# jtdaugherty/flux

Measured on AMD Instinct MI355X. Metric: Msamples/sec on demo2.yml (fixed spp), higher is better.
Workload: dtype f64

## Files before the change

flux_amd/csrc/flux_plan.h:

```cpp
#pragma once
#include <stddef.h>
#include <stdint.h>

#include "flux_device.h"

#ifndef FLUX_BLOCK_THREADS
#define FLUX_BLOCK_THREADS 64
#endif
#ifndef FLUX_WPE_SPLIT
#define FLUX_WPE_SPLIT 5
#endif
#ifndef FLUX_HITQ_MIN_TAKE
#define FLUX_HITQ_MIN_TAKE 32
#endif

namespace flux {

constexpr int kGlossExpSlots = 4;

constexpr int kQueueDoubles = 9;
constexpr int kQueueBytesPerWave = (kQueueDoubles * 64) * 8 + 2 * 64 * 4;
constexpr int kHitQDoubles = 7;
constexpr int kHitQInts = 3;
constexpr int kHitQBytesPerSlot = kHitQDoubles * 8 + kHitQInts * 4;
enum HitQField : uint32_t {
    kHitQOx = 0, kHitQOy = 2, kHitQOz = 4, kHitQDx = 6, kHitQDy = 8, kHitQDz = 10, kHitQT = 12,
    kHitQHitDepth = 14,
    kHitQSample = 15,
    kHitQList = 16,
};
constexpr uint32_t kHitQDwordsPerSlot = kHitQBytesPerSlot / 4;
constexpr uint32_t hitq_entry_dword(uint32_t C, uint32_t k) { return (C - 1u - k) * kHitQDwordsPerSlot; }
constexpr bool hitq_admits_phase_a(uint32_t C, uint32_t nhit) { return nhit + 64u <= C; }

constexpr size_t kTputEntryBytes = 24;
constexpr size_t kTputTableMaxBytes = (size_t)4 << 20;
constexpr uint32_t tput_index(uint32_t list_bits, uint32_t ml) { return (1u << list_bits) | ml; }
size_t tput_table_bytes(const RenderParams &p, int *bits = nullptr);

enum KernelCopy { kCopyStrict = 0, kCopyFast = 1, kCopyFastDiel = 2 };
KernelCopy kernel_copy(const RenderParams &p, int math);

struct LaunchPlan {
    int kernel = -1;
    unsigned block = 64;
    uint64_t blocks = 0;
    size_t lds = 0;
    unsigned waves_per_pixel = 1;
    int lds_scene = 0;
    int hq_cap = 0, hq_th = 0, hq_bits = 0;
    int copy = kCopyFast;
    int tris = 0;
    int typ = 0;
    int max32 = 0;
};
LaunchPlan plan_render(const RenderParams &p, int variant, int math);

size_t lane_stacks_lds(int math, size_t depth, bool tris, size_t bvh_stack, size_t lanes);
size_t shade_rays_lds(const RenderParams &p, int math);

}
```

flux_amd/csrc/launch_plan.cpp:

```cpp
#include <algorithm>
#include <cstdlib>

#include "flux_plan.h"
#include "../../include/flux_abi.h"

namespace flux {

KernelCopy kernel_copy(const RenderParams &p, int math) {
    if (math == FLUX_MATH_STRICT) return kCopyStrict;
    return p.has_diel ? kCopyFastDiel : kCopyFast;
}

size_t lane_stacks_lds(int math, size_t depth, bool tris, size_t bvh_stack, size_t lanes) {
    return (math == FLUX_MATH_STRICT ? depth * 4 * lanes * sizeof(double) : 0) + (tris ? bvh_stack * lanes * sizeof(int) : 0);
}

size_t shade_rays_lds(const RenderParams &p, int math) {
    return lane_stacks_lds(math, (size_t)p.max_depth, p.n_tris > 0, (size_t)p.bvh_stack, 64);
}

static bool split_typ(const RenderParams &p) {
    return p.n_sph <= 32 && p.glossy_long == 0 && p.unit_dirs == 1 && p.self_skip == 1 && p.env_short == 1 && p.n_uni == 1 &&
           p.fsph32 != nullptr && p.n_dsk == 0 && p.n_box == 0 && p.has_diel == 0 && (p.n_gloss_exp == 0 || p.gx_stride != 0);
}
// ... 7 lines not shown
    while (K * 2u <= (unsigned)FLUX_MAX_WAVES_PER_PIXEL && (uint64_t)K * 2u * FLUX_MIN_SAMPLES_PER_WAVE <= N) K *= 2u;
    return K;
}

static size_t split_scene_lds(const RenderParams &p) {
    return (size_t)hit_records(p) * sizeof(DevHitRec) + (size_t)p.n_sph * sizeof(DevScanSphere);
}
static bool split_serves(const RenderParams &p) { return p.n_tris == 0 && p.n_sph <= 64 && split_scene_lds(p) <= 16384; }

static bool plan_hitq(const RenderParams &p, unsigned K, size_t scene_lds, uint32_t &cap, uint32_t &th, int &bits) {
    if (p.glossy_long != 0 || p.has_diel != 0) return false;
    const size_t granules = (size_t)128 * K / (4 * FLUX_WPE_SPLIT);
    const size_t per_wave = granules * 1280 > scene_lds + 96 ? (granules * 1280 - scene_lds - 96) / K : 0;
    cap = (uint32_t)(per_wave / kHitQBytesPerSlot) & ~1u;
    if (const char *e = std::getenv("FLUX_SPLIT_HITQ_CAP")) cap = std::min(cap, (uint32_t)std::max(0, std::atoi(e)) & ~1u);
    th = cap > 64u + FLUX_HITQ_MIN_TAKE ? std::min(64u, cap - 64u) : FLUX_HITQ_MIN_TAKE;
    if (const char *e = std::getenv("FLUX_SPLIT_HITQ_TAKE_AT")) th = (uint32_t)std::max(1, std::min(64, std::atoi(e)));
    bits = 1;
    while ((1 << bits) < hit_records(p)) ++bits;
    return cap >= 64u + th && bits * p.max_depth <= 32;
}

size_t tput_table_bytes(const RenderParams &p, int *bits_out) {
    uint32_t cap, th;
    int bits;
    if (p.nsamp < 64u || p.max_depth < 2 || !split_serves(p) || !plan_hitq(p, waves_per_pixel(p.nsamp), split_scene_lds(p), cap, th, bits))
        return 0;
    const int list_bits = bits * (p.max_depth - 1);
    if (list_bits + 1 > 24) return 0;
    const size_t bytes = ((size_t)2 << list_bits) * kTputEntryBytes;
    if (bytes > kTputTableMaxBytes) return 0;
    if (bits_out) *bits_out = bits;
    return bytes;
}

LaunchPlan plan_render(const RenderParams &p, int variant, int math) {
    LaunchPlan L;
    L.copy = kernel_copy(p, math);
    const bool fast = L.copy != kCopyStrict;
    const uint32_t N = p.nsamp;
    const uint64_t npix = (uint64_t)p.num_rows * (uint64_t)p.img_w;
    if (npix == 0 || p.set_count <= 0) return L;
    if (variant == FLUX_KERNEL_DEFAULT) variant = N >= 256u ? FLUX_KERNEL_SPLIT : FLUX_KERNEL_REFILL;
    if (N < 64u) variant = FLUX_KERNEL_STATIC;
    const uint32_t lpp = N >= 64u ? 64u : N;
    const uint32_t ppw = 64u / lpp;
    uint64_t waves = (npix + ppw - 1) / ppw;
    if (variant != FLUX_KERNEL_STATIC && p.num_sets == (uint32_t)p.img_w)
        waves = 8ull * ((uint64_t)(p.set_count / 8) * (uint64_t)p.num_rows +
                        ((uint64_t)(p.set_count % 8) * (uint64_t)p.num_rows + 7u) / 8u);
    unsigned K = variant != FLUX_KERNEL_STATIC ? waves_per_pixel(N) : 1u;
    const bool tris = p.n_tris > 0;
    if (!fast && variant != FLUX_KERNEL_STATIC)
        while (K > 1u && lane_stacks_lds(math, (size_t)p.max_depth, tris, (size_t)p.bvh_stack, 64 * K) > 60 * 1024) K /= 2u;
    const unsigned block = (variant == FLUX_KERNEL_STATIC) ? FLUX_BLOCK_THREADS : 64u * K;
    const unsigned wpb = (variant == FLUX_KERNEL_STATIC) ? block / 64 : 1u;
    L.blocks = (waves + wpb - 1) / wpb;
    if (fast && variant != FLUX_KERNEL_STATIC && tris && p.bvh_stack > 0) {
        L.block = 64;
        size_t lds4 = (size_t)(p.bvh4_stack > 0 ? p.bvh4_stack : 1) * 64 * sizeof(int);
        const size_t scene4 = (size_t)hit_records(p) * sizeof(DevHitRec) + (size_t)p.n_mats * sizeof(DevMaterial) +
                              (size_t)p.n_sph * sizeof(DevScanSphere);
        const bool lds_scene4 = lds4 + scene4 <= 7680;
        if (lds_scene4) lds4 += scene4;
        if (p.nodes4 != nullptr && p.bvh4_stack <= FLUX_BVH_WIDE_MAX_STACK) {
            L.kernel = 4;
            L.lds = lds4;
            L.lds_scene = lds_scene4 ? 1 : 0;
            L.typ = bvh4_typ(p, lds_scene4) ? 1 : 0;
        } else {
            L.kernel = 3;
            L.lds = (size_t)p.bvh_stack * 64 * sizeof(int);
        }
        return L;
    }
    const size_t scene_lds = split_scene_lds(p);
    if (fast && variant == FLUX_KERNEL_SPLIT && split_serves(p)) {
        L.kernel = 2;
        L.block = block;
        L.waves_per_pixel = K;
        L.lds = (size_t)kQueueBytesPerWave * K + scene_lds;
        L.typ = split_typ(p) ? 1 : 0;
        L.max32 = p.n_sph <= 32 ? 1 : 0;
        uint32_t cap, th;
        int bits;
        if (plan_hitq(p, K, scene_lds, cap, th, bits)) {
            L.hq_cap = (int)cap;
            L.hq_th = (int)th;
            L.hq_bits = bits;
            L.lds = (size_t)cap * kHitQBytesPerSlot * K + scene_lds;
        }
        return L;
    }
    L.kernel = variant == FLUX_KERNEL_STATIC ? 0 : 1;
    L.block = block;
    L.waves_per_pixel = variant == FLUX_KERNEL_STATIC ? 1 : K;
    L.lds = lane_stacks_lds(math, (size_t)p.max_depth, tris, (size_t)p.bvh_stack, block);
    L.tris = tris ? 1 : 0;
    return L;
}

}
```

flux_amd/csrc/render_body.inc:

```

#undef FLUX_STAGE
#if FLUX_FAST
#define FLUX_STAGE() __builtin_amdgcn_sched_barrier(0)
#else
#define FLUX_STAGE() ((void)0)
#endif

struct Ray {
    double ox, oy, oz, dx, dy, dz;
};

typedef const __attribute__((address_space(4))) RenderParams *ParamsInKernarg;
static_assert(sizeof(DevMaterial) % 16 == 0, "the bounce-weight records behind the materials are read as double2");
__device__ __forceinline__ const RenderParams &relaunder_params(uint32_t tick) {
    ParamsInKernarg p = (ParamsInKernarg)__builtin_amdgcn_kernarg_segment_ptr();
    asm("" : "+s"(p) : "s"(tick));
    return *(const RenderParams *)p;
}

__device__ __forceinline__ unsigned long long ballot64(bool b) { return __builtin_amdgcn_ballot_w64(b); }
__device__ __forceinline__ bool any64(bool b) { return __builtin_amdgcn_ballot_w64(b) != 0ull; }
__device__ __forceinline__ bool all64(bool b) { return __builtin_amdgcn_ballot_w64(!b) == 0ull; }

typedef double flux_d2 __attribute__((ext_vector_type(2)));
// ... 765 lines not shown
#else
    return best;
#endif
}

__device__ __forceinline__ V3 to_unit_hemi(double2 p, double inv_e1) {
#if FLUX_FAST
    double sin_phi, cos_phi;
    fastmath::fsincos2pi(p.x, sin_phi, cos_phi);
    FLUX_STAGE();
    const double cos_theta = fastmath::fpow_pos(1.0 - p.y, inv_e1);
    FLUX_STAGE();
    const double sin_theta = fastmath::fsqrt(1.0 - cos_theta * cos_theta);
    return mk(sin_theta * cos_phi, sin_theta * sin_phi, cos_theta);
#else
    double phi = 2.0 * kPi * p.x;
    double sin_phi, cos_phi;
    sincos(phi, &sin_phi, &cos_phi);
    double cos_theta = pow(1.0 - p.y, inv_e1);
    double sin_theta = sqrt(1.0 - cos_theta * cos_theta);
    return normalize(mk(sin_theta * cos_phi, sin_theta * sin_phi, cos_theta));
#endif
}

__device__ __forceinline__ bool dielectric_dir(V3 n, V3 d, double ri, double u, V3 &wi) {
    const double ln = sqrt(n.x * n.x + n.y * n.y + n.z * n.z), ld = sqrt(d.x * d.x + d.y * d.y + d.z * d.z);
    const V3 nh = mk(n.x / ln, n.y / ln, n.z / ln), dh = mk(d.x / ld, d.y / ld, d.z / ld);
    double c = -(dh.x * nh.x + dh.y * nh.y + dh.z * nh.z);
    double eta = ri;
    V3 m = nh;
    if (!(c > 0.0)) {
        eta = 1.0 / ri;
        m = mk(-nh.x, -nh.y, -nh.z);
        c = -c;
    }
    const double k = 1.0 - (1.0 - c * c) / (eta * eta);
    double F = 1.0, ct = 0.0;
    if (!(k < 0.0)) {
        ct = sqrt(k);
        const double rs = (c - eta * ct) / (c + eta * ct);
        const double rp = (eta * c - ct) / (eta * c + ct);
        F = (rs * rs + rp * rp) / 2.0;
    }
    if (u <= F) {
        const double c2 = 2.0 * c;
        wi = mk(dh.x + c2 * m.x, dh.y + c2 * m.y, dh.z + c2 * m.z);
        return true;
    }
    const double a = c / eta - ct;
    wi = mk(dh.x / eta + a * m.x, dh.y / eta + a * m.y, dh.z / eta + a * m.z);
    return false;
}

struct Path {
    Ray r;
    int depth;
    int nb;
    double2 sq;
#if FLUX_FAST
    double tr, tg, tb;
    int self;
    int mat;
#endif
};
__device__ __forceinline__ int path_self(const Path &p) {
#if FLUX_FAST
    return p.self;
#else
    return -1;
#endif
}

__device__ __forceinline__ void path_begin(Path &p) {
    p.depth = 1;
    p.nb = 0;
#if FLUX_FAST
    p.tr = p.tg = p.tb = 1.0;
    p.self = -1;
    p.mat = 0;
#endif
}

#if FLUX_FAST
template <bool STATS, bool TRIS, bool TYP = false, bool FIRST = false>
__device__ __forceinline__ void fast_bounce(const RenderParams &P, Path &p, uint32_t set, uint32_t i, int hit, int slot, double t, V3 n,
                                            V3 d, V3 pt, int kind, double fr, double fg, double fb, double m_inv_e1, double ax, double az,
                                            bool unit_n, bool convex, bool is_tri, Stats &st, int cz) {
    (void)cz;
    const bool p_glossy_long = TYP ? false : P.glossy_long != 0;
    const bool p_unit_dirs = TYP ? true : P.unit_dirs != 0;
    const bool p_self_skip = TYP ? true : P.self_skip != 0;
    V3 wi;
    double scale = 1.0;
    const bool matte = kind == kMatMatte;
    FLUX_CENSUS(P, 6 + cz);
#if FLUX_DIEL
    if (!TYP && kind == kMatDielectric) {
        const char *hbase = !TRIS ? reinterpret_cast<const char *>(set_rows_of(P, set).hemi)
                                  : reinterpret_cast<const char *>(P.hemi + (size_t)set * P.max_depth * P.nsamp * 4);
        const double u = gather_global<double>(hbase, ((uint32_t)(p.depth - 1) * P.nsamp + i) * 32u + 16u);
        if (dielectric_dir(n, d, m_inv_e1, u, wi)) {
            if (STATS) st.c[10]++;
            fr = fg = fb = 1.0;
        } else {
            if (STATS) st.c[11]++;
        }
    } else
#endif
    {
        V3 w = n;
        if (!matte) {
            const double ndotwo = -dot(n, d);
            w = mk(d.x + n.x * ndotwo * 2.0, d.y + n.y * ndotwo * 2.0, d.z + n.z * ndotwo * 2.0);
        }
        if (kind == kMatReflective) {
            if (STATS) st.c[4]++;
            wi = w;
        } else {
            double hx, hy, hz;
            if (matte) {
                FLUX_CENSUS(P, 7 + cz);
                if (STATS) st.c[2]++;
                const size_t N = P.nsamp;
                const char *hbase = !TRIS ? reinterpret_cast<const char *>(set_rows_of(P, set).hemi)
                                                             : reinterpret_cast<const char *>(P.hemi + (size_t)set * P.max_depth * N * 4);
                const uint32_t hoff = ((uint32_t)(p.depth - 1) * (uint32_t)N + i) * 32u;
                const double2 hxy = gather_global_d2(hbase, hoff);
                hx = hxy.x;
                hy = hxy.y;
                hz = gather_global<double>(hbase, hoff + 16u);
                if (TRIS && is_tri) scale = 1.0 / kInvPi;
            } else {
                FLUX_CENSUS(P, 8 + cz);
                if (STATS) st.c[3]++;
                const char *gbase = !TRIS ? reinterpret_cast<const char *>(set_rows_of(P, set).gloss)
                                                             : reinterpret_cast<const char *>(P.gloss + (size_t)set * P.nsamp * 4);
                const double2 cs = gather_global_d2(gbase, i * 32u);
                double cos_theta, sin_theta;
                if (!TRIS && (TYP || P.gx_stride != 0)) {
                    const uint32_t xoff = __umul24(i, (uint32_t)P.gx_stride) + (uint32_t)gather_global<int32_t>(P.gx_off, (uint32_t)hit << 2);
                    const double2 csx = gather_global_d2(set_rows_of(P, set).glossx, xoff);
                    cos_theta = csx.x;
                    sin_theta = csx.y;
                } else {
                    cos_theta = fastmath::fexp2_tab(m_inv_e1 * gather_global<double>(gbase, i * 32u + 16u), P.exp2c);
                    sin_theta = fastmath::fsqrt(1.0 - cos_theta * cos_theta);
                }
                hx = sin_theta * cs.x;
                hy = sin_theta * cs.y;
                hz = cos_theta;
            }
            const V3 b1 = normalize(cross(mk(ax, 1.0, az), w));
            const V3 b2 = cross(b1, w);
            const double c1 = matte ? hy : hx, c2 = matte ? hx : hy;
            const V3 q = mk(c1 * b1.x + c2 * b2.x, c1 * b1.y + c2 * b2.y, c1 * b1.z + c2 * b2.z);
            const V3 hw = mk(hz * w.x, hz * w.y, hz * w.z);
            const V3 wi0 = mk(q.x + hw.x, q.y + hw.y, q.z + hw.z);
            if (matte) {
                wi = wi0;
                if (p_glossy_long) {
                    const V3 wn = normalize(wi0);
                    wi = unit_n ? wi0 : wn;
                }
            } else {
                const bool below = dot(n, wi0) < 0.0;
                wi = wi0;
                if (ballot64(below) != 0ull)
                    wi = mk(below ? hw.x - q.x : wi0.x, below ? hw.y - q.y : wi0.y, below ? hw.z - q.z : wi0.z);
                if (p_glossy_long) {
                    const double rdotwi = dot(w, wi), ndotwi = dot(n, wi);
                    const DevMaterial &Ml = P.mats[is_tri ? P.tris[slot].mat : P.frec[hit].orig_id];
                    const double e = Ml.exponent;
                    const int parity = Ml.exp_parity;
                    double lobe = fastmath::fpow_pos(fabs(rdotwi), e);
                    if (e == 0.0) lobe = 1.0;
                    if (rdotwi < 0.0) lobe = parity == 1 ? lobe : (parity == 2 ? -lobe : __builtin_nan(""));
                    if (rdotwi != rdotwi) lobe = rdotwi;
                    const double pdf = lobe * ndotwi;
                    fr *= lobe;
                    fg *= lobe;
                    fb *= lobe;
                    scale = ndotwi / pdf;
                }
            }
        }
    }
    if (p_unit_dirs) {
        const double ss = matte ? 1.0 : __builtin_fma(-0.5, dot(wi, wi), 1.5);
        wi = mk(wi.x * ss, wi.y * ss, wi.z * ss);
    }
    p.self = (p_self_skip && convex && __double2hiint(t) < 0x408f4000 && dot(n, wi) >= 0.0) ? hit : -1;
    if (FIRST) {
        p.tr = fr * scale;
        p.tg = fg * scale;
        p.tb = fb * scale;
    } else {
        p.tr *= fr * scale;
        p.tg *= fg * scale;
        p.tb *= fb * scale;
    }
    p.nb++;
    p.depth++;
    p.r.ox = pt.x;
    p.r.oy = pt.y;
    p.r.oz = pt.z;
    p.r.dx = wi.x;
    p.r.dy = wi.y;
    p.r.dz = wi.z;
}

template <bool LDS_SCENE>
__device__ __forceinline__ int analytic_hit_fields(const RenderParams &P, const Ray &r, int hit, double t, const char *frec_lds, V3 &n,
                                                   int &kind, bool &unit_n, bool &convex, double &fr, double &fg, double &fb,
                                                   double &m_inv_e1, double &ax, double &az) {
    (void)frec_lds;
    const DevHitRec R = *reinterpret_cast<const DevHitRec *>((LDS_SCENE ? frec_lds : reinterpret_cast<const char *>(P.frec)) +
                                                              (uint32_t)hit * (uint32_t)sizeof(DevHitRec));
    kind = R.mat_kind;
    unit_n = R.unit_normal != 0;
    fr = R.fr; fg = R.fg; fb = R.fb; m_inv_e1 = R.inv_e1;
    ax = R.ax; az = R.az;
    const V3 ns = mk(((r.ox - R.cx) + t * r.dx) * R.inv_rad, ((r.oy - R.cy) + t * r.dy) * R.inv_rad,
                     ((r.oz - R.cz) + t * r.dz) * R.inv_rad);
    const bool sph = R.shape_kind == kShapeSphere;
    n = mk(sph ? ns.x : R.cx, sph ? ns.y : R.cy, sph ? ns.z : R.cz);
    convex = sph && R.inv_rad > 0.0;
    return R.orig_id;
}

template <bool STATS, bool TRIS, bool LDS_SCENE = false, bool TYP = false, bool FIRST = false, bool BOUNCE = true, bool FACING = false>
__device__ __forceinline__ bool shade_hit_fast(const RenderParams &P, Path &p, uint32_t set, uint32_t i, int hit, int slot, double t,
                                               double &Lr, double &Lg, double &Lb, Stats &st, int cz, const char *frec_lds = nullptr,
                                               int facing = 0) {
    (void)frec_lds;
    (void)facing;
    (void)cz;
    int bounce = 0;
    const bool is_tri = TRIS && slot >= 0;
    const V3 d = mk(p.r.dx, p.r.dy, p.r.dz);
    const V3 pt = mk(p.r.ox + t * d.x, p.r.oy + t * d.y, p.r.oz + t * d.z);
    V3 n = mk(0.0, 0.0, 1.0);
    int kind = kMatEmissive;
    bool unit_n = true;
    bool convex = false;
    double fr = 0.0, fg = 0.0, fb = 0.0, m_inv_e1 = 0.0, ax = 0.0, az = 0.0;
    if (hit < 0) {
        Lr = P.bgr;
        Lg = P.bgg;
        Lb = P.bgb;
        if (STATS) st.c[6]++;
    } else {
        if (is_tri) {
            const DevTri &T = P.tris[slot];
            const DevMaterial &Mt = P.mats[T.mat];
            p.mat = T.mat;
            n = mk(T.nx, T.ny, T.nz);
            kind = Mt.kind;
            fr = Mt.fr; fg = Mt.fg; fb = Mt.fb; m_inv_e1 = Mt.inv_e1;
            ax = kind == kMatMatte ? 0.0034 : 0.00424;
            az = kind == kMatMatte ? 0.0071 : 0.00764;
        } else {
            p.mat = analytic_hit_fields<LDS_SCENE>(P, p.r, hit, t, frec_lds, n, kind, unit_n, convex, fr, fg, fb, m_inv_e1, ax, az);
        }
        if (kind == kMatEmissive) {
            if (STATS) st.c[5]++;
            bool front;
            if (FACING && ballot64(!facing_known(facing)) == 0ull) {
                const DevHitRec &R = *reinterpret_cast<const DevHitRec *>(frec_lds + (uint32_t)hit * (uint32_t)sizeof(DevHitRec));
                front = facing_front(facing, reinterpret_cast<const int *>(&R.inv_rad)[1]);
            } else {
                front = ((n.x * -1.0) * d.x + (n.y * -1.0) * d.y + (n.z * -1.0) * d.z) > 0.0;
            }
            Lr = fr;
            Lg = fg;
            Lb = fb;
            if (ballot64(!front) != 0ull) {
                Lr = front ? fr : 0.0;
                Lg = front ? fg : 0.0;
                Lb = front ? fb : 0.0;
            }
        } else {
            bounce = 1;
        }
    }
    asm("" : "+v"(bounce));
    if (BOUNCE && bounce) {
        fast_bounce<STATS, TRIS, TYP, FIRST>(P, p, set, i, hit, slot, t, n, d, pt, kind, fr, fg, fb, m_inv_e1, ax, az, unit_n, convex, is_tri, st,
                                            cz);
    }
    return bounce != 0;
}

template <bool STATS, bool TYP>
__device__ __forceinline__ void bounce_parked_hit(const RenderParams &P, Path &p, uint32_t set, uint32_t i, int hit, double t, Stats &st,
                                                  int cz, const char *frec_lds) {
    const V3 d = mk(p.r.dx, p.r.dy, p.r.dz);
    const V3 pt = mk(p.r.ox + t * d.x, p.r.oy + t * d.y, p.r.oz + t * d.z);
    V3 n;
    int kind;
    bool unit_n, convex;
    double fr, fg, fb, m_inv_e1, ax, az;
    p.mat = analytic_hit_fields<true>(P, p.r, hit, t, frec_lds, n, kind, unit_n, convex, fr, fg, fb, m_inv_e1, ax, az);
    fast_bounce<STATS, false, TYP, false>(P, p, set, i, hit, -1, t, n, d, pt, kind, fr, fg, fb, m_inv_e1, ax, az, unit_n, convex, false, st, cz);
}
#endif

template <bool STATS, bool TRIS, bool TWO_PHASE = false, bool LDS_SCENE = false, bool TYP = false>
__device__ __forceinline__ bool shade_hit(const RenderParams &P, Path &p, uint32_t set, uint32_t i, int hit,
                                          int slot, double t, double *stk, int stk_stride, double &Lr,
                                          double &Lg, double &Lb, Stats &st, int cz = 0, const char *frec_lds = nullptr,
                                          const char *mats_lds = nullptr) {
    (void)cz;
    (void)frec_lds;
    (void)mats_lds;
#if FLUX_FAST
    if (TWO_PHASE) return shade_hit_fast<STATS, TRIS>(P, p, set, i, hit, slot, t, Lr, Lg, Lb, st, cz);
#endif
    if (hit < 0) {
        Lr = P.bgr;
        Lg = P.bgg;
        Lb = P.bgb;
        if (STATS) st.c[6]++;
        return false;
    }
    const bool is_tri = TRIS && slot >= 0;
    const V3 d = mk(p.r.dx, p.r.dy, p.r.dz);
    const V3 pt = mk(p.r.ox + t * d.x, p.r.oy + t * d.y, p.r.oz + t * d.z);
    V3 n;
#if FLUX_FAST
    int kind;
    bool unit_n = true;
    bool convex = false;
    double fr, fg, fb, m_inv_e1, ax, az;
    if (is_tri) {
        const DevTri &T = P.tris[slot];
        const DevMaterial &Mt = LDS_SCENE ? *reinterpret_cast<const DevMaterial *>(mats_lds + (uint32_t)T.mat * (uint32_t)sizeof(DevMaterial))
                                          : P.mats[T.mat];
        p.mat = T.mat;
        n = mk(T.nx, T.ny, T.nz);
        kind = Mt.kind;
        fr = Mt.fr; fg = Mt.fg; fb = Mt.fb; m_inv_e1 = Mt.inv_e1;
        ax = kind == kMatMatte ? 0.0034 : 0.00424;
        az = kind == kMatMatte ? 0.0071 : 0.00764;
    } else {
        const DevHitRec R = *reinterpret_cast<const DevHitRec *>((LDS_SCENE ? frec_lds : reinterpret_cast<const char *>(P.frec)) +
                                                                  (uint32_t)hit * (uint32_t)sizeof(DevHitRec));
        kind = R.mat_kind;
        p.mat = R.orig_id;
        unit_n = R.unit_normal != 0;
        fr = R.fr; fg = R.fg; fb = R.fb; m_inv_e1 = R.inv_e1;
        ax = R.ax; az = R.az;
        const V3 ns = mk(((p.r.ox - R.cx) + t * d.x) * R.inv_rad, ((p.r.oy - R.cy) + t * d.y) * R.inv_rad,
                         ((p.r.oz - R.cz) + t * d.z) * R.inv_rad);
        const bool sph = R.shape_kind == kShapeSphere;
        n = mk(sph ? ns.x : R.cx, sph ? ns.y : R.cy, sph ? ns.z : R.cz);
        convex = sph && R.inv_rad > 0.0;
    }
    if (kind == kMatEmissive) {
        if (STATS) st.c[5]++;
        const bool front = ((n.x * -1.0) * d.x + (n.y * -1.0) * d.y + (n.z * -1.0) * d.z) > 0.0;
        Lr = front ? fr : 0.0;
        Lg = front ? fg : 0.0;
        Lb = front ? fb : 0.0;
        return false;
    }
#else
    const DevShape *S = P.shapes + (is_tri ? 0 : hit);
// ... 462 lines not shown
template <bool TYP>
__device__ __forceinline__ void scan_shapes_primary(const RenderParams &P, const Ray &r, unsigned long long cand_mask,
                                                    unsigned long long in_mask, double in_t0, bool valid, unsigned long long valid_m,
                                                    int &best, double &tb) {
    (void)valid;
    (void)valid_m;
    int best_id = -1;
    const double tmin = P.t_min;
    int j0 = 0;
    if (P.n_pln > 0) {
        const DevScanPlane &S = P.fpln[0];
        const double num = (S.px - r.ox) * S.nx + (S.py - r.oy) * S.ny + (S.pz - r.oz) * S.nz;
        const double den = r.dx * S.nx + r.dy * S.ny + r.dz * S.nz;
        const double t = num / den;
        best = t > tmin ? P.n_sph : -1;
        best_id = S.id;
        tb = t;
        j0 = 1;
    }
    for (int j = j0; j < P.n_pln; ++j) {
        const DevScanPlane &S = P.fpln[j];
        const double num = (S.px - r.ox) * S.nx + (S.py - r.oy) * S.ny + (S.pz - r.oz) * S.nz;
        const double den = r.dx * S.nx + r.dy * S.ny + r.dz * S.nz;
        const double t = num / den;
        if (t > tmin && (best < 0 || t < tb)) {
            best = P.n_sph + j;
            best_id = S.id;
            tb = t;
        }
    }
    if (!TYP) {
        scan_disks(P, r, tmin, best, best_id, tb);
        scan_boxes(P, r, tmin, best, best_id, tb);
    }
    const double rs = 1.0, ux = r.dx, uy = r.dy, uz = r.dz, len = 1.0;
    const bool zflat = r.dz == 0.0, any_zflat = any64(zflat);
    for (int pass = 0; pass < 2; ++pass) {
        unsigned long long todo = pass == 0 ? (cand_mask & ~in_mask) : in_mask;
        if (pass == 1 && todo && (valid_m & ~(ballot64(best >= 0) & ballot64(tb <= in_t0))) == 0ull) todo &= todo - 1;
        while (todo) {
            const int k = __builtin_ctzll(todo);
            todo &= todo - 1;
            const DevScanSphere S = P.fsph[k];
            FLUX_TRIP(P, 13);
            FLUX_CENSUS(P, 1);
            const double tx = r.ox - S.px, ty = r.oy - S.py, tz = r.oz - S.pz;
            const double hb = sphere_hb(tx, ty, tz, ux, uy, uz);
            const double c = __builtin_fma(tx, tx, __builtin_fma(ty, ty, __builtin_fma(tz, tz, -S.rr)));
            if (pass == 1) {
                const double tu = tb * len;
                const double g = __builtin_fma(tu, __builtin_fma(2.0, hb, tu), c);
                if ((valid_m & ~(ballot64(best >= 0) & ballot64(g < -1e-7 * S.rr))) == 0ull) continue;
            }
            const double dq = __builtin_fma(hb, hb, -c);
            const double e = fastmath::fsqrt_nonneg(__builtin_fmax(dq, 0.0));
            double t = (-hb - e) * rs;
            if (!(t > tmin)) t = (-hb + e) * rs;
            bool ok = dq >= 0.0 && t > tmin;
            if (any_zflat) {
                if (zflat && box_z_nan_miss(P, r, k)) ok = false;
            }
            if (ok) {
                bool take = best < 0 || t < tb;
                if (!take && t == tb) take = best >= P.n_sph ? P.frec[k].orig_id < best_id : k < best;
                if (take) {
                    best = k;
                    tb = t;
                }
            }
        }
    }
}

__device__ __forceinline__ double lds_dword_pair(const uint32_t *p) { return __hiloint2double((int)p[1], (int)p[0]); }
__device__ __forceinline__ void lds_dword_pair_store(uint32_t *p, double v) {
    p[0] = (uint32_t)__double2loint(v);
    p[1] = (uint32_t)__double2hiint(v);
}

__device__ __forceinline__ uint32_t *hitq_entry(uint32_t *pool, uint32_t C, uint32_t k) {
    return reinterpret_cast<uint32_t *>(reinterpret_cast<char *>(pool) + __umul24(C - 1u - k, (uint32_t)kHitQBytesPerSlot));
}

template <bool STATS, bool MAX32, bool TYP, bool HQ = false>
__global__ __launch_bounds__(64 * FLUX_MAX_WAVES_PER_PIXEL, FLUX_WPE_SPLIT) void render_split_kernel(const RenderParams P0, int hq_cap, int hq_th,
                                                                                                  int hq_bits) {
    (void)hq_cap;
    (void)hq_th;
    (void)hq_bits;
    const RenderParams &P = P0;
    extern __shared__ double lds_stack[];
    __shared__ double part[FLUX_MAX_WAVES_PER_PIXEL][3];
    const int tid = threadIdx.x;
    const uint32_t lane = tid & 63;
    const uint32_t N = P.nsamp;
    const uint32_t K = blockDim.x >> 6, sub = (uint32_t)__builtin_amdgcn_readfirstlane(tid >> 6);
    const uint32_t s_lo = (uint32_t)((uint64_t)N * sub / K), s_hi = (uint32_t)((uint64_t)N * (sub + 1) / K);
    const int n_rec = TYP ? P.n_sph + P.n_pln + P.n_dsk : hit_records(P);
    const size_t scene_lds_bytes = (size_t)n_rec * sizeof(DevHitRec) + (size_t)P.n_sph * sizeof(DevScanSphere);
    double *q = lds_stack + scene_lds_bytes / 8 + (size_t)sub * (HQ ? (size_t)hq_cap * kHitQBytesPerSlot / 8 : kQueueBytesPerWave / 8);
    int *qi = reinterpret_cast<int *>(q + (size_t)kQueueDoubles * 64);
    const char *const frec_lds = reinterpret_cast<const char *>(lds_stack);
    const char *const fsph_lds = frec_lds + (size_t)n_rec * sizeof(DevHitRec);
    {
        uint32_t *dst = reinterpret_cast<uint32_t *>(const_cast<char *>(frec_lds));
        const uint32_t nrec_w = (uint32_t)n_rec * (uint32_t)(sizeof(DevHitRec) / 4), nsph_w = (uint32_t)P.n_sph * 8u;
        const uint32_t *src_r = reinterpret_cast<const uint32_t *>(P.frec), *src_s = reinterpret_cast<const uint32_t *>(P.fsph);
        for (uint32_t w = (uint32_t)tid; w < nrec_w; w += blockDim.x) dst[w] = src_r[w];
        for (uint32_t w = (uint32_t)tid; w < nsph_w; w += blockDim.x) dst[nrec_w + w] = src_s[w];
        __syncthreads();
    }
    const uint64_t wave = blockIdx.x;
    int lrow = 0, col = 0, row = 0;
    uint32_t set = 0;
    uint64_t pixel = 0;
    const bool wave_on = map_wave(P, wave, lrow, col, row, set, pixel);
    set = (uint32_t)__builtin_amdgcn_readfirstlane((int)set);
    col = __builtin_amdgcn_readfirstlane(col);
    row = __builtin_amdgcn_readfirstlane(row);

    Stats st = {};
    double sr = 0.0, sg = 0.0, sb = 0.0;
    if (HQ && wave_on) {
        unsigned long long cand_mask, in_mask;
        double in_t0;
        pixel_sphere_mask(P, row, col, lane, cand_mask, in_mask, in_t0);
        const uint32_t C = (uint32_t)hq_cap, H = (uint32_t)hq_th;
        const uint32_t bmask = (1u << hq_bits) - 1u;
        const DevHitRec *const recs = reinterpret_cast<const DevHitRec *>(frec_lds);
        uint32_t *const pool = reinterpret_cast<uint32_t *>(q);
        uint32_t next = s_lo;
        uint32_t nhit = 0;
        constexpr int kDeadDepth = 0x7fffffff;
        for (;;) {
            const RenderParams &P = relaunder_params(next + nhit);
            uint32_t set_p = set;
            unsigned long long cand_p = cand_mask, in_p = in_mask;
            asm("" : "+s"(set_p) : "s"(next));
            asm("" : "+s"(cand_p), "+s"(in_p) : "s"(next));
            Path p;
            path_begin(p);
            p.depth = kDeadDepth;
            p.sq = make_double2(0.5, 0.5);
            uint32_t i = 0;
            uint32_t ml = 0;
            const bool run_a = next < s_hi && nhit < H && hitq_admits_phase_a(C, nhit);
            if (run_a) {
                FLUX_TRIP(P, 12);
                FLUX_CENSUS(P, 0);
                const uint32_t ia = next + lane;
                const bool valid = ia < s_hi;
                const unsigned long long valid_m = ballot64(ia < s_hi);
                next = (s_hi - next) > 64u ? next + 64u : s_hi;
                bool cont = false;
                const double2 *pix = set_rows_of(P, set_p).pix;
                const double2 *disc = set_rows_of(P, set_p).disc;
                const char *pxc_b = reinterpret_cast<const char *>(P.pxc);
                const PixelConsts PX = PixelConsts{*reinterpret_cast<const double *>(pxc_b + ((uint32_t)col << 3)),
                                                   *reinterpret_cast<const double *>(pxc_b + ((uint32_t)(P.img_w + row) << 3)), P.fwx, P.fwy, P.fwz};
                {
                    const uint32_t ic = ia < s_hi ? ia : s_hi - 1u;
                    p.sq = gather_global_d2(pix, ic << 4);
                    p.r = primary_ray_px(P, PX, p.sq, gather_global_d2(disc, ic << 4));
                    if (STATS && valid) {
                        st.c[0]++;
                        st.c[1]++;
                    }
                }
                int hit = -1;
                double t = 0.0;
                scan_shapes_primary<TYP>(P, p.r, cand_p, in_p, in_t0, valid, valid_m, hit, t);
                p.depth = 1;
                if (valid) {
                    double Lr, Lg, Lb;
                    FLUX_CENSUS(P, 2);
                    cont = shade_hit_fast<STATS, false, true, TYP, true>(P, p, set_p, ia, hit, -1, t, Lr, Lg, Lb, st, 3, frec_lds);
                    if (cont && p.depth > P.max_depth) {
                        cont = false;
                        Lr = Lg = Lb = 0.0;
                        if (STATS) st.c[7]++;
                    }
                    if (!cont) {
                        fold_path(p, nullptr, 0, Lr, Lg, Lb);
                        sr += Lr;
                        sg += Lg;
                        sb += Lb;
                    }
                }
                i = ia;
                ml = (uint32_t)hit;
                if (!cont) p.depth = kDeadDepth;
            }
            if (nhit) {
                const unsigned long long freemask = ballot64(p.depth == kDeadDepth);
                const uint32_t nfree = (uint32_t)__popcll(freemask);
                const uint32_t take = nfree < nhit ? nfree : nhit;
                if (!run_a || take >= H || !(next < s_hi && hitq_admits_phase_a(C, nhit))) {
                    const uint32_t rank = __builtin_amdgcn_mbcnt_hi((uint32_t)(freemask >> 32),
                                                                    __builtin_amdgcn_mbcnt_lo((uint32_t)freemask, 0u));
                    if (p.depth == kDeadDepth && rank < take) {
                        FLUX_CENSUS(P, 15);
                        const uint32_t *e = hitq_entry(pool, C, nhit - 1u - rank);
                        p.r.ox = lds_dword_pair(e + kHitQOx);
                        p.r.oy = lds_dword_pair(e + kHitQOy);
                        p.r.oz = lds_dword_pair(e + kHitQOz);
                        p.r.dx = lds_dword_pair(e + kHitQDx);
                        p.r.dy = lds_dword_pair(e + kHitQDy);
                        p.r.dz = lds_dword_pair(e + kHitQDz);
                        const double t = lds_dword_pair(e + kHitQT);
                        const int hd = (int)e[kHitQHitDepth];
                        i = e[kHitQSample];
                        const int hit = hd & 0xffff;
                        p.depth = hd >> 16;
                        ml = e[kHitQList];
                        const uint32_t list_bits = __umul24((uint32_t)(p.depth - 1), (uint32_t)hq_bits);
                        if (P.tput != nullptr) {
                            const uint32_t off = __umul24(tput_index(list_bits, ml), (uint32_t)kTputEntryBytes);
                            p.tr = gather_global<double>(P.tput, off);
                            p.tg = gather_global<double>(P.tput, off + 8u);
                            p.tb = gather_global<double>(P.tput, off + 16u);
                        } else {
                            const DevHitRec &R0 = recs[ml & bmask];
                            p.tr = R0.fr;
                            p.tg = R0.fg;
                            p.tb = R0.fb;
#pragma unroll 1
                            for (int k = 1; k < p.depth - 1; ++k) {
                                const DevHitRec &Rk = recs[(ml >> (k * hq_bits)) & bmask];
                                p.tr *= Rk.fr;
                                p.tg *= Rk.fg;
                                p.tb *= Rk.fb;
                            }
                        }
                        ml |= (uint32_t)hit << list_bits;
                        bounce_parked_hit<STATS, TYP>(P, p, set_p, i, hit, t, st, 6, frec_lds);
                    }
                    nhit -= take;
                }
            }
            if (__builtin_expect((nhit | (s_hi - next)) == 0u, 0)) {
                if (!any64(p.depth != kDeadDepth)) break;
            }
            FLUX_TRIP(P, 10);
            const bool live = p.depth != kDeadDepth;
            const bool trace = p.depth <= P.max_depth;
            double Lr = 0.0, Lg = 0.0, Lb = 0.0;
            bool cont = false;
            int hit = -1;
            double t = 0.0;
            if (trace) {
                FLUX_CENSUS(P, 3);
                if (STATS) st.c[1]++;
                const float ofx = (float)p.r.ox, ofy = (float)p.r.oy, ofz = (float)p.r.oz;
                const float oo32 = __builtin_fmaf(ofz, ofz, __builtin_fmaf(ofy, ofy, ofx * ofx));
                int facing;
                if (__builtin_expect((ballot64(p.r.dz == 0.0) | ballot64(!(oo32 < 0.999e6f))) != 0ull, 0))
                    scan_shapes_fast<true, true, MAX32, TYP, 1, true>(P, p.r, p.self, hit, t, nullptr, fsph_lds, &facing);
                else
                    scan_shapes_fast<true, true, MAX32, TYP, 0, true>(P, p.r, p.self, hit, t, nullptr, fsph_lds, &facing);
// ... 29 lines not shown
        double in_t0;
        pixel_sphere_mask(P, row, col, lane, cand_mask, in_mask, in_t0);

#ifdef FLUX_DEBUG_CLOCK
        long long lap_store[8] = {0, 0, 0, 0, 0, 0, 0, (long long)__builtin_readcyclecounter()};
        long long *lap = lap_store;
#else
        long long *lap = nullptr;
#endif
        uint32_t next = s_lo;
        uint32_t qcount = 0;
        uint32_t i = 0;
        constexpr int kDeadDepth = 0x7fffffff;
        Path p;
        path_begin(p);
        p.depth = kDeadDepth;
        p.sq = make_double2(0.0, 0.0);
        p.r = Ray{0, 0, 0, 0, 0, 1};
        for (;;) {
            const RenderParams &P = relaunder_params(next + qcount);
            uint32_t set_p = set;
            unsigned long long cand_p = cand_mask, in_p = in_mask;
            asm("" : "+s"(set_p) : "s"(next));
            asm("" : "+s"(cand_p), "+s"(in_p) : "s"(next));
            auto pop = [&]() {
                const unsigned long long freemask = ballot64(p.depth == kDeadDepth);
                if (!freemask || !qcount) return;
                const uint32_t nfree = (uint32_t)__popcll(freemask);
                const uint32_t take = nfree < qcount ? nfree : qcount;
                const uint32_t rank = __builtin_amdgcn_mbcnt_hi((uint32_t)(freemask >> 32),
                                                                __builtin_amdgcn_mbcnt_lo((uint32_t)freemask, 0u));
                if (p.depth == kDeadDepth && rank < take) {
                    const uint32_t slot = qcount - 1u - rank;
                    p.r.ox = q[0 * 64 + slot];
                    p.r.oy = q[1 * 64 + slot];
                    p.r.oz = q[2 * 64 + slot];
                    p.r.dx = q[3 * 64 + slot];
                    p.r.dy = q[4 * 64 + slot];
                    p.r.dz = q[5 * 64 + slot];
                    p.tr = q[6 * 64 + slot];
                    p.tg = q[7 * 64 + slot];
                    p.tb = q[8 * 64 + slot];
                    i = (uint32_t)qi[slot];
                    p.self = qi[64 + slot];
                    p.depth = 2;
                    p.nb = 1;
                }
                qcount -= take;
            };
            pop();
            lap_stamp(lap, 0);
            if (next < s_hi && any64(p.depth == kDeadDepth)) {
                FLUX_TRIP(P, 12);
                FLUX_CENSUS(P, 0);
                const uint32_t ia = next + lane;
                const bool valid = ia < s_hi;
                const unsigned long long valid_m = ballot64(ia < s_hi);
                next = (s_hi - next) > 64u ? next + 64u : s_hi;
                bool cont = false;
                Path pa;
                path_begin(pa);
                pa.sq = make_double2(0.5, 0.5);
                pa.r = Ray{0, 0, 0, 0, 0, 1};
                const double2 *pix = set_rows_of(P, set_p).pix;
                const double2 *disc = set_rows_of(P, set_p).disc;
                const char *pxc_b = reinterpret_cast<const char *>(P.pxc);
                const PixelConsts PX = PixelConsts{*reinterpret_cast<const double *>(pxc_b + ((uint32_t)col << 3)),
                                                   *reinterpret_cast<const double *>(pxc_b + ((uint32_t)(P.img_w + row) << 3)), P.fwx, P.fwy, P.fwz};
                {
                    const uint32_t ic = ia < s_hi ? ia : s_hi - 1u;
                    pa.sq = gather_global_d2(pix, ic << 4);
                    pa.r = primary_ray_px(P, PX, pa.sq, gather_global_d2(disc, ic << 4));
                    if (STATS && valid) {
                        st.c[0]++;
                        st.c[1]++;
                    }
                }
                int hit = -1;
                double t = 0.0;
                scan_shapes_primary<TYP>(P, pa.r, cand_p, in_p, in_t0, valid, valid_m, hit, t);
                if (valid) {
                    double Lr, Lg, Lb;
                    FLUX_CENSUS(P, 2);
                    cont = shade_hit_fast<STATS, false, true, TYP, true>(P, pa, set_p, ia, hit, -1, t, Lr, Lg, Lb, st, 3, frec_lds);
                    if (cont && pa.depth > P.max_depth) {
                        cont = false;
                        Lr = Lg = Lb = 0.0;
                        if (STATS) st.c[7]++;
                    }
                    if (!cont) {
                        fold_path(pa, nullptr, 0, Lr, Lg, Lb);
                        sr += Lr;
                        sg += Lg;
                        sb += Lb;
                    }
                }
                const unsigned long long qmask = ballot64(cont);
                if (cont) {
                    const uint32_t slot = __builtin_amdgcn_mbcnt_hi((uint32_t)(qmask >> 32),
                                                                    __builtin_amdgcn_mbcnt_lo((uint32_t)qmask, 0u));
                    q[0 * 64 + slot] = pa.r.ox;
                    q[1 * 64 + slot] = pa.r.oy;
                    q[2 * 64 + slot] = pa.r.oz;
                    q[3 * 64 + slot] = pa.r.dx;
                    q[4 * 64 + slot] = pa.r.dy;
                    q[5 * 64 + slot] = pa.r.dz;
                    q[6 * 64 + slot] = pa.tr;
                    q[7 * 64 + slot] = pa.tg;
                    q[8 * 64 + slot] = pa.tb;
                    qi[slot] = (int)ia;
                    qi[64 + slot] = pa.self;
                }
                qcount = (uint32_t)__popcll(qmask);
                lap_stamp(lap, 1);
                pop();
                lap_stamp(lap, 0);
            }
            if (__builtin_expect((qcount | (s_hi - next)) == 0u, 0)) {
                if (!any64(p.depth != kDeadDepth)) break;
            }
            FLUX_TRIP(P, 10);
            const bool live = p.depth != kDeadDepth;
            const bool trace = p.depth <= P.max_depth;
            double Lr = 0.0, Lg = 0.0, Lb = 0.0;
            bool cont = false;
            if (trace) {
                FLUX_CENSUS(P, 3);
                if (STATS) st.c[1]++;
                int hit = -1;
                double t = 0.0;
                const float ofx = (float)p.r.ox, ofy = (float)p.r.oy, ofz = (float)p.r.oz;
                const float oo32 = __builtin_fmaf(ofz, ofz, __builtin_fmaf(ofy, ofy, ofx * ofx));
                if (__builtin_expect((ballot64(p.r.dz == 0.0) | ballot64(!(oo32 < 0.999e6f))) != 0ull, 0))
                    scan_shapes_fast<true, true, MAX32, TYP, 1>(P, p.r, p.self, hit, t, lap, fsph_lds);
                else
                    scan_shapes_fast<true, true, MAX32, TYP, 0>(P, p.r, p.self, hit, t, lap, fsph_lds);
                cont = shade_hit_fast<STATS, false, true, TYP>(P, p, set_p, i, hit, -1, t, Lr, Lg, Lb, st, 0, frec_lds);
            }
            if (live && !cont) {
                if (STATS && !trace) st.c[7]++;
                fold_path(p, nullptr, 0, Lr, Lg, Lb);
                sr += Lr;
                sg += Lg;
                sb += Lb;
                p.depth = kDeadDepth;
            }
            lap_stamp(lap, 5);
        }
#ifdef FLUX_DEBUG_CLOCK
        if (P.stats && lane == 0)
            for (int k = 0; k < 6; ++k) atomicAdd(P.stats + 10 + k, (unsigned long long)lap[k]);
#endif
    }
    const RenderParams &PE = P;
    if (K == 1) {
        finish_pixel(PE, wave_on, lane, 0u, 64u, pixel, sr, sg, sb);
    } else {
        double r, g, b;
        wave_sum3(sr, sg, sb, r, g, b);
        if (lane == 0) {
            part[sub][0] = r;
            part[sub][1] = g;
            part[sub][2] = b;
        }
        __syncthreads();
        if (sub == 0) {
            double tr = 0.0, tg = 0.0, tb = 0.0;
// ... 621 lines not shown
    const int tid = threadIdx.x;
    const int k = blockIdx.x * 64 + tid;
    double *stk = lds_stack + tid;
    int *tstack = bvh_stack_base(lds_stack, P, 64) + tid;
    if (k >= n) return;
    Stats st = {};
    Path p;
    path_begin(p);
    p.depth = depth;
    p.sq = P.pix[(size_t)set * P.nsamp + index];
    p.r = Ray{rays[6 * k], rays[6 * k + 1], rays[6 * k + 2], rays[6 * k + 3], rays[6 * k + 4], rays[6 * k + 5]};
    {
        double t = 0.0;
        int slot = -1;
        const int hit = scene_hit<false, TRIS>(P, p.r, path_self(p), t, slot, tstack, 64, st);
        int id = hit;
#if FLUX_FAST
        if (hit >= 0 && !(TRIS && slot >= 0)) id = P.frec[hit].orig_id;
#endif
        out_hit[k] = id;
        out_t[k] = hit >= 0 ? t : 0.0;
    }
    double Lr, Lg, Lb;
    while (shade_level<false, TRIS>(P, p, set, index, stk, 64, tstack, Lr, Lg, Lb, st)) {
    }
    fold_path(p, stk, 64, Lr, Lg, Lb);
    out_rgb[3 * k] = Lr;
    out_rgb[3 * k + 1] = Lg;
    out_rgb[3 * k + 2] = Lb;
}

static hipError_t launch_shade_rays_impl(const RenderParams &p, size_t lds, const double *d_rays, int n, int depth, uint32_t set,
                                         uint32_t index, double *d_rgb, int *d_hit, double *d_t, hipStream_t stream) {
    if (n <= 0) return hipSuccess;
    const dim3 g((unsigned)((n + 63) / 64)), b(64);
    if (p.n_tris > 0) shade_rays_kernel<true><<<g, b, lds, stream>>>(p, d_rays, n, depth, set, index, d_rgb, d_hit, d_t);
    else shade_rays_kernel<false><<<g, b, lds, stream>>>(p, d_rays, n, depth, set, index, d_rgb, d_hit, d_t);
    return hipGetLastError();
}

static hipError_t launch_render_impl(const LaunchPlan &L, const RenderParams &p, hipStream_t stream) {
    if (L.blocks > 0x7fffffffull) return hipErrorInvalidValue;
    const bool tris = L.tris != 0;
    const bool stats = p.stats != nullptr;
    const dim3 g((unsigned)L.blocks), b(L.block);
    const size_t lds = L.lds;
#define FLUX_LAUNCH(K)                                                     \
    do {                                                                   \
        if (stats && tris) K<true, true><<<g, b, lds, stream>>>(p);        \
        else if (stats) K<true, false><<<g, b, lds, stream>>>(p);          \
        else if (tris) K<false, true><<<g, b, lds, stream>>>(p);           \
        else K<false, false><<<g, b, lds, stream>>>(p);                    \
    } while (0)
#if FLUX_FAST
    if (L.kernel == 3) {
        if (stats) render_bvh_kernel<true><<<g, b, lds, stream>>>(p);
        else render_bvh_kernel<false><<<g, b, lds, stream>>>(p);
        return hipGetLastError();
    }
    if (L.kernel == 4) {
        if (L.typ) {
#if FLUX_DIEL
            return hipErrorInvalidValue;
#else
            if (stats) render_bvh4_kernel<true, true, true><<<g, b, lds, stream>>>(p);
            else render_bvh4_kernel<false, true, true><<<g, b, lds, stream>>>(p);
#endif
        } else if (L.lds_scene) {
            if (stats) render_bvh4_kernel<true, true, false><<<g, b, lds, stream>>>(p);
            else render_bvh4_kernel<false, true, false><<<g, b, lds, stream>>>(p);
        } else {
            if (stats) render_bvh4_kernel<true, false, false><<<g, b, lds, stream>>>(p);
            else render_bvh4_kernel<false, false, false><<<g, b, lds, stream>>>(p);
        }
        return hipGetLastError();
    }
    if (L.kernel == 2) {
        const int c = L.hq_cap, h = L.hq_th, bits = L.hq_bits;
        const bool hq = L.hq_cap > 0;
        RenderParams ps = p;
        if (!hq || ps.tput_bits != bits) ps.tput = nullptr;
#define FLUX_LAUNCH_SPLIT(MAX32, TYP, HQ)                                                                      \
    do {                                                                                                       \
        if (stats) render_split_kernel<true, MAX32, TYP, HQ><<<g, b, lds, stream>>>(ps, c, h, bits);           \
        else render_split_kernel<false, MAX32, TYP, HQ><<<g, b, lds, stream>>>(ps, c, h, bits);                \
    } while (0)
#if FLUX_DIEL
        if (L.typ || hq) return hipErrorInvalidValue;
#else
        if (L.typ) {
            if (hq) FLUX_LAUNCH_SPLIT(true, true, true);
            else FLUX_LAUNCH_SPLIT(true, true, false);
            return hipGetLastError();
        }
        if (hq) {
            if (L.max32) FLUX_LAUNCH_SPLIT(true, false, true);
            else FLUX_LAUNCH_SPLIT(false, false, true);
            return hipGetLastError();
        }
#endif
        if (L.max32) FLUX_LAUNCH_SPLIT(true, false, false);
        else FLUX_LAUNCH_SPLIT(false, false, false);
#undef FLUX_LAUNCH_SPLIT
        return hipGetLastError();
    }
#endif
    if (L.kernel == 0)
        FLUX_LAUNCH(render_static_kernel);
    else
        FLUX_LAUNCH(render_refill_kernel);
#undef FLUX_LAUNCH
    return hipGetLastError();
}
```

Before: 53980.

## Add wave-uniform primary-hit shading path with scalar hit-record loads

When every lane in a wave hits the same primitive on the primary ray, shading takes a specialised path. That path reads the hit record through a scalar (constant address space) pointer and uses a simplified bounce with fewer selects and skipped normalisation for matte surfaces. The aim is to replace per-lane LDS/global gathers and divergent selects with scalar loads and leaner arithmetic. The cost is an extra ballot and readfirstlane per primary hit, more code and register pressure, and a second instantiation of the shading code. An environment variable can turn it off.

```diff
diff --git a/flux_amd/csrc/flux_plan.h b/flux_amd/csrc/flux_plan.h
--- a/flux_amd/csrc/flux_plan.h
+++ b/flux_amd/csrc/flux_plan.h
@@ -53,6 +53,7 @@
     int tris = 0;
     int typ = 0;
     int max32 = 0;
+    int uniform_a = 1;
 };
 LaunchPlan plan_render(const RenderParams &p, int variant, int math);
 
diff --git a/flux_amd/csrc/launch_plan.cpp b/flux_amd/csrc/launch_plan.cpp
--- a/flux_amd/csrc/launch_plan.cpp
+++ b/flux_amd/csrc/launch_plan.cpp
@@ -113,6 +113,7 @@
         L.lds = (size_t)kQueueBytesPerWave * K + scene_lds;
         L.typ = split_typ(p) ? 1 : 0;
         L.max32 = p.n_sph <= 32 ? 1 : 0;
+        if (const char *e = std::getenv("FLUX_SPLIT_UNIFORM_A")) L.uniform_a = std::atoi(e) != 0 ? 1 : 0;
         uint32_t cap, th;
         int bits;
         if (plan_hitq(p, K, scene_lds, cap, th, bits)) {
diff --git a/flux_amd/csrc/render_body.inc b/flux_amd/csrc/render_body.inc
--- a/flux_amd/csrc/render_body.inc
+++ b/flux_amd/csrc/render_body.inc
@@ -871,7 +871,7 @@
 }
 
 #if FLUX_FAST
-template <bool STATS, bool TRIS, bool TYP = false, bool FIRST = false>
+template <bool STATS, bool TRIS, bool TYP = false, bool FIRST = false, bool UNI = false>
 __device__ __forceinline__ void fast_bounce(const RenderParams &P, Path &p, uint32_t set, uint32_t i, int hit, int slot, double t, V3 n,
                                             V3 d, V3 pt, int kind, double fr, double fg, double fb, double m_inv_e1, double ax, double az,
                                             bool unit_n, bool convex, bool is_tri, Stats &st, int cz) {
@@ -907,6 +907,7 @@
             wi = w;
         } else {
             double hx, hy, hz;
+            double c1u = 0.0, c2u = 0.0;
             if (matte) {
                 FLUX_CENSUS(P, 7 + cz);
                 if (STATS) st.c[2]++;
@@ -918,6 +919,8 @@
                 hx = hxy.x;
                 hy = hxy.y;
                 hz = gather_global<double>(hbase, hoff + 16u);
+                c1u = hy;
+                c2u = hx;
                 if (TRIS && is_tri) scale = 1.0 / kInvPi;
             } else {
                 FLUX_CENSUS(P, 8 + cz);
@@ -938,16 +941,20 @@
                 hx = sin_theta * cs.x;
                 hy = sin_theta * cs.y;
                 hz = cos_theta;
+                c1u = hx;
+                c2u = hy;
             }
             const V3 b1 = normalize(cross(mk(ax, 1.0, az), w));
             const V3 b2 = cross(b1, w);
-            const double c1 = matte ? hy : hx, c2 = matte ? hx : hy;
+            const double c1 = UNI ? c1u : (matte ? hy : hx), c2 = UNI ? c2u : (matte ? hx : hy);
             const V3 q = mk(c1 * b1.x + c2 * b2.x, c1 * b1.y + c2 * b2.y, c1 * b1.z + c2 * b2.z);
             const V3 hw = mk(hz * w.x, hz * w.y, hz * w.z);
             const V3 wi0 = mk(q.x + hw.x, q.y + hw.y, q.z + hw.z);
             if (matte) {
                 wi = wi0;
-                if (p_glossy_long) {
+                if (UNI) {
+                    if (p_glossy_long && !unit_n) wi = normalize(wi0);
+                } else if (p_glossy_long) {
                     const V3 wn = normalize(wi0);
                     wi = unit_n ? wi0 : wn;
                 }
@@ -974,11 +981,23 @@
             }
         }
     }
-    if (p_unit_dirs) {
+    if (UNI) {
+        if (p_unit_dirs && !matte) {
+            double ww = dot(wi, wi);
+            asm("" : "+v"(ww));
+            const double ss = __builtin_fma(-0.5, ww, 1.5);
+            wi = mk(wi.x * ss, wi.y * ss, wi.z * ss);
+        }
+    } else if (p_unit_dirs) {
         const double ss = matte ? 1.0 : __builtin_fma(-0.5, dot(wi, wi), 1.5);
         wi = mk(wi.x * ss, wi.y * ss, wi.z * ss);
     }
-    p.self = (p_self_skip && convex && __double2hiint(t) < 0x408f4000 && dot(n, wi) >= 0.0) ? hit : -1;
+    if (UNI) {
+        p.self = -1;
+        if (p_self_skip && convex) p.self = (__double2hiint(t) < 0x408f4000 && dot(n, wi) >= 0.0) ? hit : -1;
+    } else {
+        p.self = (p_self_skip && convex && __double2hiint(t) < 0x408f4000 && dot(n, wi) >= 0.0) ? hit : -1;
+    }
     if (FIRST) {
         p.tr = fr * scale;
         p.tg = fg * scale;
@@ -998,11 +1017,28 @@
     p.r.dz = wi.z;
 }
 
-template <bool LDS_SCENE>
+typedef const __attribute__((address_space(4))) DevHitRec *HitRecScalar;
+template <bool LDS_SCENE, bool UNI = false>
 __device__ __forceinline__ int analytic_hit_fields(const RenderParams &P, const Ray &r, int hit, double t, const char *frec_lds, V3 &n,
                                                    int &kind, bool &unit_n, bool &convex, double &fr, double &fg, double &fb,
                                                    double &m_inv_e1, double &ax, double &az) {
     (void)frec_lds;
+    if (UNI) {
+        const HitRecScalar Ru = (HitRecScalar)(reinterpret_cast<uintptr_t>(P.frec) + (uint32_t)hit * (uint32_t)sizeof(DevHitRec));
+        kind = Ru->mat_kind;
+        unit_n = Ru->unit_normal != 0;
+        fr = Ru->fr; fg = Ru->fg; fb = Ru->fb; m_inv_e1 = Ru->inv_e1;
+        ax = Ru->ax; az = Ru->az;
+        const double cx = Ru->cx, cy = Ru->cy, cz = Ru->cz, inv_rad = Ru->inv_rad;
+        if (Ru->shape_kind == kShapeSphere) {
+            n = mk(((r.ox - cx) + t * r.dx) * inv_rad, ((r.oy - cy) + t * r.dy) * inv_rad, ((r.oz - cz) + t * r.dz) * inv_rad);
+            convex = inv_rad > 0.0;
+        } else {
+            n = mk(cx, cy, cz);
+            convex = false;
+        }
+        return Ru->orig_id;
+    }
     const DevHitRec R = *reinterpret_cast<const DevHitRec *>((LDS_SCENE ? frec_lds : reinterpret_cast<const char *>(P.frec)) +
                                                               (uint32_t)hit * (uint32_t)sizeof(DevHitRec));
     kind = R.mat_kind;
@@ -1017,7 +1053,8 @@
     return R.orig_id;
 }
 
-template <bool STATS, bool TRIS, bool LDS_SCENE = false, bool TYP = false, bool FIRST = false, bool BOUNCE = true, bool FACING = false>
+template <bool STATS, bool TRIS, bool LDS_SCENE = false, bool TYP = false, bool FIRST = false, bool BOUNCE = true, bool FACING = false,
+          bool UNI = false>
 __device__ __forceinline__ bool shade_hit_fast(const RenderParams &P, Path &p, uint32_t set, uint32_t i, int hit, int slot, double t,
                                                double &Lr, double &Lg, double &Lb, Stats &st, int cz, const char *frec_lds = nullptr,
                                                int facing = 0) {
@@ -1049,7 +1086,7 @@
             ax = kind == kMatMatte ? 0.0034 : 0.00424;
             az = kind == kMatMatte ? 0.0071 : 0.00764;
         } else {
-            p.mat = analytic_hit_fields<LDS_SCENE>(P, p.r, hit, t, frec_lds, n, kind, unit_n, convex, fr, fg, fb, m_inv_e1, ax, az);
+            p.mat = analytic_hit_fields<LDS_SCENE, UNI>(P, p.r, hit, t, frec_lds, n, kind, unit_n, convex, fr, fg, fb, m_inv_e1, ax, az);
         }
         if (kind == kMatEmissive) {
             if (STATS) st.c[5]++;
@@ -1069,9 +1106,15 @@
                 Lb = front ? fb : 0.0;
             }
         } else {
+            if (UNI) {
+                if (BOUNCE) fast_bounce<STATS, TRIS, TYP, FIRST, true>(P, p, set, i, hit, slot, t, n, d, pt, kind, fr, fg, fb, m_inv_e1, ax, az,
+                                                                       unit_n, convex, is_tri, st, cz);
+                return true;
+            }
             bounce = 1;
         }
     }
+    if (UNI) return false;
     asm("" : "+v"(bounce));
     if (BOUNCE && bounce) {
         fast_bounce<STATS, TRIS, TYP, FIRST>(P, p, set, i, hit, slot, t, n, d, pt, kind, fr, fg, fb, m_inv_e1, ax, az, unit_n, convex, is_tri, st,
@@ -1700,9 +1743,24 @@
     return reinterpret_cast<uint32_t *>(reinterpret_cast<char *>(pool) + __umul24(C - 1u - k, (uint32_t)kHitQBytesPerSlot));
 }
 
+template <bool STATS, bool TYP, bool UNIFORM_A>
+__device__ __forceinline__ bool shade_primary_hits(const RenderParams &P, Path &p, uint32_t set, uint32_t ia, int hit, double t, double &Lr,
+                                                   double &Lg, double &Lb, Stats &st, const char *frec_lds, int uni_a) {
+    if (UNIFORM_A) {
+        const int hu = __builtin_amdgcn_readfirstlane(hit);
+        if (uni_a != 0 && ballot64(hit != hu) == 0ull) {
+            FLUX_CENSUS(P, 16);
+            return shade_hit_fast<STATS, false, true, TYP, true, true, false, true>(P, p, set, ia, hu, -1, t, Lr, Lg, Lb, st, 3, frec_lds);
+        }
+    }
+    FLUX_CENSUS(P, 17);
+    return shade_hit_fast<STATS, false, true, TYP, true>(P, p, set, ia, hit, -1, t, Lr, Lg, Lb, st, 3, frec_lds);
+}
+constexpr bool split_uniform_a(bool TYP, bool HQ) { return HQ || TYP; }
+
 template <bool STATS, bool MAX32, bool TYP, bool HQ = false>
 __global__ __launch_bounds__(64 * FLUX_MAX_WAVES_PER_PIXEL, FLUX_WPE_SPLIT) void render_split_kernel(const RenderParams P0, int hq_cap, int hq_th,
-                                                                                                  int hq_bits) {
+                                                                                                  int hq_bits, int uni_a) {
     (void)hq_cap;
     (void)hq_th;
     (void)hq_bits;
@@ -1792,7 +1850,7 @@
                 if (valid) {
                     double Lr, Lg, Lb;
                     FLUX_CENSUS(P, 2);
-                    cont = shade_hit_fast<STATS, false, true, TYP, true>(P, p, set_p, ia, hit, -1, t, Lr, Lg, Lb, st, 3, frec_lds);
+                    cont = shade_primary_hits<STATS, TYP, split_uniform_a(TYP, HQ)>(P, p, set_p, ia, hit, t, Lr, Lg, Lb, st, frec_lds, uni_a);
                     if (cont && p.depth > P.max_depth) {
                         cont = false;
                         Lr = Lg = Lb = 0.0;
@@ -1988,7 +2046,7 @@
                 if (valid) {
                     double Lr, Lg, Lb;
                     FLUX_CENSUS(P, 2);
-                    cont = shade_hit_fast<STATS, false, true, TYP, true>(P, pa, set_p, ia, hit, -1, t, Lr, Lg, Lb, st, 3, frec_lds);
+                    cont = shade_primary_hits<STATS, TYP, split_uniform_a(TYP, HQ)>(P, pa, set_p, ia, hit, t, Lr, Lg, Lb, st, frec_lds, uni_a);
                     if (cont && pa.depth > P.max_depth) {
                         cont = false;
                         Lr = Lg = Lb = 0.0;
@@ -2776,8 +2834,8 @@
         if (!hq || ps.tput_bits != bits) ps.tput = nullptr;
 #define FLUX_LAUNCH_SPLIT(MAX32, TYP, HQ)                                                                      \
     do {                                                                                                       \
-        if (stats) render_split_kernel<true, MAX32, TYP, HQ><<<g, b, lds, stream>>>(ps, c, h, bits);           \
-        else render_split_kernel<false, MAX32, TYP, HQ><<<g, b, lds, stream>>>(ps, c, h, bits);                \
+        if (stats) render_split_kernel<true, MAX32, TYP, HQ><<<g, b, lds, stream>>>(ps, c, h, bits, L.uniform_a);  \
+        else render_split_kernel<false, MAX32, TYP, HQ><<<g, b, lds, stream>>>(ps, c, h, bits, L.uniform_a);   \
     } while (0)
 #if FLUX_DIEL
         if (L.typ || hq) return hipErrorInvalidValue;
```

After: 54940 (median of 6 runs). 1.02x the previous value.
